# george-tyler-315-incline/ggml-neon-opt

Hardware: AMD Instinct MI355X
Metric: tg128 tok/s + Q4_K GEMV achieved-HBM-GB/s, TinyLlama-1.1B Q4_K_M @1 GPU (higher is better)
Workload: dtype q4_K/q6_K x q8_K (u4/u6*i8 dot4 -> i32, f32 combine); 1 GPU; tinyllama-1.1b Q4_K_M tg2221: full decode graph, token i at position i of a fresh f16 KV cache; parallelism=replicas x1, hipgraph=True

## Files before the change

ggml-neon-opt_amd/csrc/kq_backend.hip:

```cpp
#include <algorithm>
#include <dlfcn.h>
#include <stdio.h>
#include <stdlib.h>
#include <string.h>

#include <rccl/rccl.h>

#include <string>
#include <vector>

#include "kq_common.h"
#include "kq_internal.h"
#include "kq_plan.h"

using kq::attn_batch_desc_of;
using kq::attn_desc_of;
using kq::f_of;
using kq::Launch;
using kq::LaunchKind;
using kq::nelem;

struct mi355x_backend {
    int device = 0;
    hipStream_t stream = nullptr;
// ... 539 lines not shown
        }
        tb.stride = stride;
        tb.key.swap(key);
        b->ly_tabs.push_back(std::move(tb));
    }
    return MI355X_OK;
}

int reserve_attn_cells(mi355x_backend *b, mi355x_tensor *const *nodes, const std::vector<Launch> &launches) {
    for (const Launch &l : launches) {
        const mi355x_tensor *t = nodes[l.first];
        if (l.kind != LaunchKind::Node || t->op != MI355X_OP_ATTN_DECODE) continue;
        const int64_t T = t->src[0]->ne[1];
        mi355x_attn_desc d = {};
        attn_desc_of(t, d);
        if (T > 1) d.rope_row = 0;
        kq::AttnArgs a = {};
        if (kq::attn_args_from(&d, a) == MI355X_OK && kq::attn_cells_reserve(a, b->stream, (int)T) != MI355X_OK)
            return MI355X_E_WORKSPACE;
    }
    return MI355X_OK;
}

int capture_and_launch(mi355x_backend *b, mi355x_tensor *const *nodes, int n_nodes, const std::vector<Launch> &launches) {
    std::vector<uint64_t> key = kq::graph_key_of(nodes, n_nodes);
    mi355x_backend::Captured *c = find_graph(b, key);
    if (!c) {
        if (hipStreamBeginCapture(b->stream, hipStreamCaptureModeThreadLocal) != hipSuccess)
            return MI355X_E_UNSUPPORTED;
        const int rc = enqueue(b, nodes, launches);
        hipGraph_t g = nullptr;
        const hipError_t ec = hipStreamEndCapture(b->stream, &g);
        if (rc || ec != hipSuccess) {
            if (g) hipGraphDestroy(g);
            return rc ? rc : (int)ec;
        }
        hipGraphExec_t ge = nullptr;
        if (hipGraphInstantiate(&ge, g, nullptr, nullptr, 0) != hipSuccess) {
            hipGraphDestroy(g);
            return MI355X_E_UNSUPPORTED;
        }
        if (b->graphs.size() == kMaxGraphs) {
            hipStreamSynchronize(b->stream);
            destroy_captured(b->graphs.front());
            b->graphs.erase(b->graphs.begin());
        }
        mi355x_backend::Captured nc;
        nc.key.swap(key);
// ... 223 lines not shown
}

int mi355x_backend_set_fusion(mi355x_backend_t b, int enable) {
    return b ? toggle(b, b->fuse, enable) : MI355X_E_INVAL;
}

int mi355x_backend_graph_compute(mi355x_backend_t b, mi355x_tensor *const *nodes, int n_nodes, int use_graph) {
    if (!b || (n_nodes > 0 && !nodes) || n_nodes < 0) return MI355X_E_INVAL;
    DeviceGuard dg(b->device);
    if (use_graph && !b->graphs.empty()) {
        const std::vector<uint64_t> key = kq::graph_key_of(nodes, n_nodes);
        if (mi355x_backend::Captured *c = find_graph(b, key)) {
            const hipError_t e = hipGraphLaunch(c->exec, b->stream);
            return e == hipSuccess ? 0 : (int)e;
        }
    }
    int rc = ensure_workspace(b, nodes, n_nodes);
    if (rc) return rc;
    const std::vector<Launch> launches = kq::plan_launches(plan_opts(b), nodes, n_nodes);
    if ((rc = ensure_attn_oproj_buffer(b, nodes, launches))) return rc;
    if ((rc = ensure_layer_blocks(b, launches))) return rc;
    if ((rc = ensure_layer_tables(b, launches))) return rc;
    if ((rc = reserve_attn_cells(b, nodes, launches))) return rc;
    return use_graph ? capture_and_launch(b, nodes, n_nodes, launches) : enqueue(b, nodes, launches);
}

}
```

ggml-neon-opt_amd/csrc/kq_internal.h:

```cpp
#pragma once

#include <string>
#include <tuple>

#include <hip/hip_ext.h>

#include "kq_common.h"

namespace kq {

int device_ok();
int num_cus();
constexpr size_t kMaxLds = 160 * 1024;
constexpr size_t kTargetLds = 80 * 1024;
void allow_lds(const void *fn, size_t lds);
int resident_wgs(const void *fn, size_t lds);
uint64_t *diag_stamps(int64_t *cap);
enum Knob {
    KNOB_GEMV_DIAG,
    KNOB_GEMV_RING,
    KNOB_GEMV_PRE0,
    KNOB_GEMV_PF,
    KNOB_GEMV_XMODE,
    KNOB_GEMV_SMALL_MB,
// ... 125 lines not shown
int launch_mmf_multi(int type, int n_mat, const void *const *w, const int64_t *N, const size_t *row_stride,
                     float *const *y, const int64_t *y_col_stride, int64_t K, uint8_t *ws, size_t ws_size, int64_t M,
                     hipStream_t stream, const float *res = nullptr, int64_t res_col_stride = 0);
size_t mmf_workspace(int64_t N, int64_t M, int64_t nb);
struct MmqKv {
    int kind[4];
    const int32_t *pos;
    const float *rope;
    uint16_t *k_cache, *v_cache;
    int n_ctx, hd;
};
int launch_mmq_multi(const int *types, int n_mat, const void *const *w, const int64_t *N, const size_t *row_stride,
                     float *const *y, const int64_t *y_col_stride, int64_t K, const uint8_t *xq, int64_t M,
                     hipStream_t stream, const MmqKv *kv = nullptr);

int launch_rows_prologue_dbg(int pro, const float *x, const float *x2, float eps, int nb, int waves, uint8_t *out,
                             hipStream_t s);
int launch_rms_norm_q8L(const float *x, const float *w, void *yq, int64_t n, int64_t nrows, float eps, hipStream_t s);
int launch_swiglu_q8L(const float *g, const float *u, void *yq, int64_t n, int64_t nrows, hipStream_t s);

int launch_rms_norm(const float *x, const float *w, float *y, int64_t n, int64_t nrows, float eps, hipStream_t s);
int launch_binary(int op, const float *a, const float *b, float *y, int64_t n, hipStream_t s,
                  int64_t nb = 0);
int launch_attn_prompt(const AttnArgs &a, int n_tok, hipStream_t s);
int attn_cells_reserve(const AttnArgs &a, hipStream_t stream, int n_tok = 1);
bool attn_prompt_q8_ok(const AttnArgs &a);
int launch_swiglu(const float *g, const float *u, float *y, int64_t n, hipStream_t s);
int attn_args_from(const mi355x_attn_desc *d, AttnArgs &a);
int launch_attn(const AttnArgs &a, hipStream_t s);
bool attn_group_ok(const AttnArgs &a, int nwaves);
size_t attn_group_bytes(const AttnArgs &a, int nwaves);
int attn_impl();
size_t attn_lds(int hd, int n_ctx);
size_t attn_prompt_lds(int hd, int n_ctx);
void *attn_cells_buffer(size_t bytes, hipStream_t stream, bool may_alloc);
int launch_kv_store(const AttnArgs &a, int n_tok, hipStream_t s);

constexpr int kAttnStreamMaxCtx = 131072;
int attn_stream_mode();
bool attn_size_refused(const AttnArgs &a);
bool attn_stream_applies(const AttnArgs &a);
bool attn_stream_prompt_applies(const AttnArgs &a);
size_t attn_stream_workspace(const AttnArgs &a, int n_tok);
int launch_attn_stream(const AttnArgs &a, hipStream_t s);
int launch_attn_stream_prompt(const AttnArgs &a, int n_tok, hipStream_t s);

// ... 18 lines not shown
```

ggml-neon-opt_amd/csrc/kq_ops.hip:

```cpp
#include <math.h>
#include <stdlib.h>
#include <string.h>

#include <atomic>
#include <mutex>
#include <vector>

#include <hip/hip_ext.h>

#include "kq_common.h"
#include "kq_internal.h"
#include "kq_attn_device.h"
#include "kq_attn_head.h"
#include "kq_device.h"
#include "kq_ops_device.h"
#include "kq_rows_device.h"

#ifndef KQ_ATTN_BATCH_CTX
#define KQ_ATTN_BATCH_CTX 256
#endif
#ifndef KQ_ATTN_OSC1
#define KQ_ATTN_OSC1 0
#endif

namespace kq {

constexpr int GETROWS_STAGE = ((15 + 8 * 210 + 15) / 16) * 16;
__global__ void __launch_bounds__(256) kq_get_rows(int type, const uint8_t *__restrict__ table, int64_t k,
                                                   int64_t row_stride, int64_t n_rows,
                                                   const int32_t *__restrict__ ids, float *__restrict__ out) {
    __shared__ __attribute__((aligned(16))) uint8_t stage[GETROWS_STAGE];
    const int64_t r = blockIdx.y;
    const int64_t e0 = ((int64_t)blockIdx.x * 256 + threadIdx.x) * 8;
    const bool live = e0 < k;
    const int64_t id = ids[r];
    float *y = out + r * k + e0;
    if (id < 0 || id >= n_rows) {
        if (live) {
#pragma unroll
            for (int i = 0; i < 8; ++i) y[i] = __builtin_nanf("");
        }
        return;
    }
    const uint8_t *grow = table + id * row_stride;
    if (type == MI355X_TYPE_F32) {
        if (live) {
            const float *s = (const float *)grow + e0;
#pragma unroll
            for (int i = 0; i < 8; ++i) y[i] = s[i];
        }
        return;
    }
    const int bsz = block_bytes(type);
    const int64_t b0 = (int64_t)blockIdx.x * 8;
    const int64_t left = k / QK - b0;
    const int nblk = (int)(left < 8 ? left : 8);
    const uint8_t *src = grow + b0 * bsz;
    const uint32_t mis = (uint32_t)((uintptr_t)src & 15u);
    const int ng = (int)((mis + (uint32_t)(nblk * bsz) + 15u) / 16u);
// ... 24 lines not shown
        const uint8_t *qh = blk + 16 + l0;
#pragma unroll
        for (int i = 0; i < 8; ++i) {
            const int hb = q5 ? ((qh[i] >> (2 * j + h)) & 1) << 4 : 0;
            y[i] = __builtin_fmaf(d1, (float)(((q[i] >> (4 * h)) & 0xF) + hb), -m1);
        }
    } else {
        const uint8_t *blk = row + b * 210;
        const float d = h2f((uint16_t)(blk[208] | (blk[209] << 8)));
        const int half = e / 128, rr = e % 128, quarter = rr / 32, l0 = rr % 32;
        const uint8_t *ql = blk + 64 * half, *qh = blk + 128 + 32 * half;
        const int8_t *sc = (const int8_t *)(blk + 192) + 8 * half;
#pragma unroll
        for (int i = 0; i < 8; ++i) {
            const int l = l0 + i;
            int q;
            if (quarter == 0) q = (ql[l] & 0xF) | (((qh[l] >> 0) & 3) << 4);
            else if (quarter == 1) q = (ql[l + 32] & 0xF) | (((qh[l] >> 2) & 3) << 4);
            else if (quarter == 2) q = (ql[l] >> 4) | (((qh[l] >> 4) & 3) << 4);
            else q = (ql[l + 32] >> 4) | (((qh[l] >> 6) & 3) << 4);
            y[i] = d * (float)sc[l / 16 + 2 * quarter] * (float)(q - 32);
        }
    }
}

__global__ void __launch_bounds__(256) kq_rms_norm(const float *__restrict__ x, const float *__restrict__ w,
                                                   float *__restrict__ y, int64_t n, float eps) {
    extern __shared__ __attribute__((aligned(16))) double sb_sum[];
    const int64_t row = blockIdx.x;
    const float *xr = x + row * n;
    float *yr = y + row * n;
    const int nb = (int)(n / QK);
    const int rid = threadIdx.x >> 4, l = threadIdx.x & 15;
    for (int b0 = 0; b0 < nb; b0 += 16) {
        const int b = b0 + rid;
        double s = 0.0;
        if (b < nb) {
            float v[16];
            const float4 *p = (const float4 *)(xr + (int64_t)b * QK + 16 * l);
#pragma unroll
            for (int k = 0; k < 4; ++k) {
                const float4 t = p[k];
                v[4 * k] = t.x, v[4 * k + 1] = t.y, v[4 * k + 2] = t.z, v[4 * k + 3] = t.w;
            }
            s = sumsq16(v);
        }
// ... 1031 lines not shown
    if (rc) return rc;
    if (group) {
        if (gsz == 8 && tpw > 1) KQ_PROMPT_GROUP_LAUNCH(128, 8, KQ_PROMPT_TPW)
        if (gsz == 4 && tpw > 1) KQ_PROMPT_GROUP_LAUNCH(128, 4, KQ_PROMPT_TPW)
        if (gsz == 8) KQ_PROMPT_GROUP_LAUNCH(128, 8, 1)
        if (gsz == 4) KQ_PROMPT_GROUP_LAUNCH(128, 4, 1)
        KQ_PROMPT_GROUP_LAUNCH(128, 0, 1)
    }
#undef KQ_PROMPT_GROUP_LAUNCH
    allow_lds((const void *)kq_attn_prompt<128>, lds);
    return timed_launch("kq::kq_attn_prompt<128>", 0.0, kq_attn_prompt<128>, ga, dim3(256), lds, s, a);
}

int check_attn(const AttnArgs &a) {
    if (!a.q || !a.k || !a.v || !a.pos || !a.rope_table || !a.k_cache || !a.v_cache || !a.out) return MI355X_E_INVAL;
    if (a.head_dim != 64 && a.head_dim != 128) return MI355X_E_UNSUPPORTED;
    if (a.n_head <= 0 || a.n_head_kv <= 0 || a.n_head % a.n_head_kv) return MI355X_E_INVAL;
    if (a.n_ctx < 32 || a.n_ctx % 32) return MI355X_E_UNSUPPORTED;
    if (((uintptr_t)a.k_cache & 15u) || ((uintptr_t)a.v_cache & 15u)) return MI355X_E_INVAL;
    if (attn_size_refused(a) && !attn_stream_applies(a)) return MI355X_E_UNSUPPORTED;
    return MI355X_OK;
}

uint64_t ops_selector_key() {
    return (uint64_t)(uint32_t)attn_impl() | ((uint64_t)(uint32_t)g_prompt_impl.load() << 8) |
           ((uint64_t)(uint32_t)attn_stream_mode() << 16);
}

}

using namespace kq;

extern "C" {

int mi355x_get_rows(int type, const void *table, int64_t ne0, size_t row_stride, int64_t n_rows, const int32_t *ids,
                    int64_t n_ids, float *dst, void *stream) {
    if (!table || !ids || !dst || ne0 <= 0 || n_ids < 0 || n_rows < 0) return MI355X_E_INVAL;
    if (type != MI355X_TYPE_F32 && type != MI355X_TYPE_Q4_K && type != MI355X_TYPE_Q5_K && type != MI355X_TYPE_Q6_K)
        return MI355X_E_UNSUPPORTED;
    if (ne0 % (type == MI355X_TYPE_F32 ? 8 : QK)) return MI355X_E_INVAL;
    if (row_stride < mi355x_row_size(type, ne0) && type != MI355X_TYPE_F32) return MI355X_E_INVAL;
    if (n_ids == 0) return MI355X_OK;
    if (!device_ok()) return MI355X_E_NODEVICE;
    const dim3 grid((unsigned)((ne0 / 8 + 255) / 256), (unsigned)n_ids);
    return timed_launch("kq::kq_get_rows", (double)n_ids * (ne0 * 4.0 + (double)mi355x_row_size(type, ne0)),
                        kq_get_rows, grid, dim3(256), 0, (hipStream_t)stream, type, (const uint8_t *)table, ne0,
// ... 133 lines not shown
```

ggml-neon-opt_amd/csrc/kq_plan.h:

```cpp
#pragma once

#include <string.h>

#include <vector>

#include "kq_common.h"
#include "kq_internal.h"

namespace kq {

enum class LaunchKind {
    Node,
    GemvRun,
    PrefillPrologue,
    MmAdd,
    MmMulti,
    AttnOproj,
    Layer,
};

struct Launch {
    int first, count;
    LaunchKind kind = LaunchKind::Node;
    const mi355x_tensor *q8_of = nullptr;
// ... 13 lines not shown
    bool fuse, attn_oproj, layer_engine;
    const void *workspace;
    size_t workspace_size;
};

inline int64_t nelem(const mi355x_tensor *t) { return t->ne[0] * t->ne[1] * t->ne[2] * t->ne[3]; }
inline float f_of(int32_t bits) {
    float f;
    memcpy(&f, &bits, 4);
    return f;
}
inline const mi355x_tensor *other_operand(const mi355x_tensor *add, const mi355x_tensor *mm) {
    return add->src[0] == mm ? add->src[1] : add->src[1] == mm ? add->src[0] : nullptr;
}

std::vector<Launch> plan_launches(const PlanOpts &o, mi355x_tensor *const *nodes, int n);
bool batched_mm_shares(const PlanOpts &o, const mi355x_tensor *t);
bool attn_feeds_batched_mm(const PlanOpts &o, const mi355x_tensor *t, const Launch &next, mi355x_tensor *const *nodes);
bool kv_epilogue(mi355x_tensor *const *nodes, const Launch &l, const Launch &next, MmqKv &kv);
void attn_desc_of(const mi355x_tensor *t, mi355x_attn_desc &a);
void attn_batch_desc_of(const mi355x_tensor *t, mi355x_attn_batch_desc &d);
std::vector<uint64_t> graph_key_of(mi355x_tensor *const *nodes, int n_nodes);
bool supports_op(const mi355x_tensor *op);

}
```

ggml-neon-opt_amd/csrc/kq_plan.hip:

```cpp
#include "kq_plan.h"

namespace kq {
namespace {

bool is_kquant(int t) { return t == MI355X_TYPE_Q4_K || t == MI355X_TYPE_Q5_K || t == MI355X_TYPE_Q6_K; }

struct Span {
    uintptr_t lo = 0, hi = 0;
};
Span span_of(const mi355x_tensor *t) {
    Span s;
    if (!t || !t->data) return s;
    const int64_t blck = is_kquant(t->type) ? MI355X_QK_K : 1;
    uint64_t bytes = (uint64_t)(t->ne[0] / blck) * t->nb[0];
    for (int d = 1; d < 4; ++d)
        if (t->ne[d] > 1) bytes += (uint64_t)(t->ne[d] - 1) * t->nb[d];
    s.lo = (uintptr_t)t->data;
    s.hi = s.lo + (uintptr_t)bytes;
    return s;
}

std::vector<int> count_readers(mi355x_tensor *const *nodes, int n) {
    std::vector<int> r(n, 0);
    std::vector<Span> out(n);
// ... 450 lines not shown
    key.reserve((size_t)n_nodes * 16 + 2);
    key.push_back(api_selector_key());
    key.push_back(ops_selector_key());
    for (int i = 0; i < n_nodes; ++i) {
        const mi355x_tensor *t = nodes[i];
        key.push_back((uint64_t)(uintptr_t)t->data);
        key.push_back((uint64_t)t->op);
        key.push_back((uint64_t)t->flags);
        for (int d = 0; d < 4; ++d) key.push_back((uint64_t)t->ne[d]);
        for (int d = 0; d < 8; ++d) key.push_back((uint64_t)(uint32_t)t->op_params[d]);
        for (int s = 0; s < MI355X_MAX_SRC; ++s) {
            const mi355x_tensor *u = t->src[s];
            if (!u) { key.push_back(0); continue; }
            key.push_back((uint64_t)(uintptr_t)u->data);
            key.push_back((uint64_t)u->type);
            for (int d = 0; d < 4; ++d) key.push_back((uint64_t)u->ne[d]);
            for (int d = 0; d < 4; ++d) key.push_back((uint64_t)u->nb[d]);
        }
        for (int d = 0; d < 4; ++d) key.push_back((uint64_t)t->nb[d]);
    }
    return key;
}

bool supports_op(const mi355x_tensor *op) {
    if (!op) return false;
    switch (op->op) {
        case MI355X_OP_NONE:
            return true;
        case MI355X_OP_MUL_MAT: {
            const mi355x_tensor *w = op->src[0], *x = op->src[1];
            if (!w || !x) return false;
            if (!is_kquant(w->type) || x->type != MI355X_TYPE_F32 || op->type != MI355X_TYPE_F32) return false;
            if (w->ne[0] % MI355X_QK_K || w->ne[0] != x->ne[0]) return false;
            if (w->ne[2] != 1 || w->ne[3] != 1 || x->ne[2] != 1 || x->ne[3] != 1) return false;
            if (op->ne[0] != w->ne[1] || op->ne[1] != x->ne[1]) return false;
            if (x->nb[0] != 4 || op->nb[0] != 4) return false;
            return w->nb[0] == mi355x_row_size(w->type, MI355X_QK_K);
        }
        case MI355X_OP_GET_ROWS: {
            const mi355x_tensor *w = op->src[0], *ids = op->src[1];
            if (!w || !ids || ids->type != MI355X_TYPE_I32 || !ids->data || ids->nb[0] != 4 || !contig_f32(op))
                return false;
            if (w->type != MI355X_TYPE_F32 && !is_kquant(w->type)) return false;
            if (op->ne[1] > 1 && op->nb[1] != (size_t)op->ne[0] * 4) return false;
            return op->ne[0] == w->ne[0] && op->ne[1] == ids->ne[0] && w->ne[0] % MI355X_QK_K == 0;
        }
// ... 66 lines not shown
```

ggml-neon-opt_amd/ggml_mi355x/__init__.py:

```python
from __future__ import annotations

import ctypes
import os

HERE = os.path.dirname(os.path.abspath(__file__))
PKG_ROOT = os.path.dirname(HERE)
LIB_PATH = os.environ.get("MI355X_LIB") or os.path.join(PKG_ROOT, "lib", "libggml_mi355x.so")

TYPE_F32, TYPE_F16, TYPE_Q4_K, TYPE_Q5_K, TYPE_Q6_K, TYPE_Q8_K, TYPE_I32 = 0, 1, 12, 13, 14, 15, 26
TYPE_I64 = 27
QK_K = 256
BLOCK_BYTES = {TYPE_Q4_K: 144, TYPE_Q5_K: 176, TYPE_Q6_K: 210, TYPE_Q8_K: 292}
TYPE_NAMES = {TYPE_Q4_K: "q4_K", TYPE_Q5_K: "q5_K", TYPE_Q6_K: "q6_K", TYPE_Q8_K: "q8_K", TYPE_F32: "f32"}
MAX_FUSED = 4
OP_NONE, OP_MUL_MAT, OP_GET_ROWS, OP_RMS_NORM, OP_MUL, OP_ADD, OP_SWIGLU, OP_ROPE, OP_ATTN_DECODE, OP_ALL_GATHER, \
    OP_ALL_REDUCE = range(11)
OP_ATTN_BATCH = 11
MAX_SRC = 10
FLAG_OUTPUT = 1
E_OK, E_INVAL, E_UNSUPPORTED, E_WORKSPACE, E_NODEVICE, E_COMM, E_LAYER = 0, -1, -2, -3, -4, -6, -7
PRO_NONE, PRO_RMS_NORM, PRO_SWIGLU = 0, 1, 2
EPI_NONE, EPI_SWIGLU = 0, 1
ATTN_GROUP, ATTN_HEAD, ATTN_SPLIT = 0, 1, 2
ATTN_PATH_HEAD, ATTN_PATH_HEAD_BATCH, ATTN_PATH_SPLIT4, ATTN_PATH_SPLIT8, ATTN_PATH_CELLS, ATTN_PATH_GROUP, ATTN_PATH_KD1 = range(7)
ATTN_PATH_STREAM = 7
MMQ_AUTO, MMQ_TILE64, MMQ_TILE128, MMQ_TILE128W, MMQ_TILE64W, MMQ_TILE128X, MMQ_TILE192 = 0, 1, 2, 3, 4, 5, 6
PREFILL_EXACT, PREFILL_F16, PREFILL_F16_ALL = 0, 1, 2

EXPORTED_SYMBOLS = (
    "mi355x_row_size", "mi355x_version", "mi355x_device_available",
    "mi355x_quantize_row_q8_K", "mi355x_vec_dot_q4_K_q8_K", "mi355x_vec_dot_q5_K_q8_K",
    "mi355x_vec_dot_q6_K_q8_K", "mi355x_quantize_q8_K", "mi355x_mul_mat_workspace_size",
    "mi355x_mul_mat", "mi355x_mul_mat_q8", "mi355x_gemv_fused", "mi355x_debug_block_partials", "mi355x_debug_stream",
    "mi355x_backend_init", "mi355x_backend_free", "mi355x_backend_name", "mi355x_backend_stream",
    "mi355x_backend_alloc", "mi355x_backend_free_buffer", "mi355x_backend_set_tensor",
    "mi355x_backend_get_tensor", "mi355x_backend_synchronize", "mi355x_backend_supports_op",
    "mi355x_backend_graph_compute", "mi355x_timing_enable", "mi355x_timing_read", "mi355x_diag_stamps",
    "mi355x_gemv_fused_workspace_size", "mi355x_gemv_impl",
    "mi355x_gguf_open", "mi355x_gguf_close", "mi355x_gguf_version", "mi355x_gguf_alignment",
    "mi355x_gguf_data_offset", "mi355x_gguf_n_tensors", "mi355x_gguf_find_tensor", "mi355x_gguf_get_tensor",
    "mi355x_gguf_tensor_data", "mi355x_gguf_upload", "mi355x_gguf_n_kv", "mi355x_gguf_find_key",
    "mi355x_gguf_key", "mi355x_gguf_kv_type", "mi355x_gguf_get_int", "mi355x_gguf_get_float",
    "mi355x_gguf_get_str", "mi355x_gguf_arr_n",
    "mi355x_gemv_ext_workspace_size", "mi355x_gemv_fused_ext", "mi355x_backend_set_fusion",
    "mi355x_get_rows", "mi355x_rms_norm", "mi355x_add", "mi355x_mul", "mi355x_swiglu",
    "mi355x_rope_table_size", "mi355x_rope_table", "mi355x_rope", "mi355x_attn_decode", "mi355x_attn_path",
    "mi355x_comm_id_size", "mi355x_comm_get_unique_id", "mi355x_backend_set_comm", "mi355x_backend_comm_world",
    "mi355x_backend_set_comm_loopback", "mi355x_lower_ggml_graph", "mi355x_attn_impl",
    "mi355x_mmq_impl",
    "mi355x_prefill_precision",
    "mi355x_gemv_waves",
    "mi355x_debug_knob",
    "mi355x_device_count", "mi355x_device_ordinal", "mi355x_device_memory", "mi355x_backend_memset", "mi355x_backend_set_attn_oproj",
    "mi355x_backend_set_layer_engine", "mi355x_backend_layer_error",
    "mi355x_attn_prompt",
    "mi355x_attn_prompt_impl", "mi355x_attn_stream",
    "mi355x_attn_batch", "mi355x_attn_batch_path",
    "mi355x_rows_prologue_plan", "mi355x_rows_stream_plan", "mi355x_debug_rows_prologue",
    "mi355x_debug_rows_plan",
)


class Mi355xError(RuntimeError):
    pass


class GemvDesc(ctypes.Structure):
    _fields_ = [("type", ctypes.c_int), ("w", ctypes.c_void_p), ("n_rows", ctypes.c_int64),
                ("row_stride", ctypes.c_size_t), ("y", ctypes.c_void_p)]


class LaunchTiming(ctypes.Structure):
    _fields_ = [("kernel", ctypes.c_char * 96), ("bytes", ctypes.c_double), ("ms", ctypes.c_float)]


class Tensor(ctypes.Structure):
    pass


Tensor._fields_ = [("type", ctypes.c_int), ("op", ctypes.c_int), ("ne", ctypes.c_int64 * 4),
                   ("nb", ctypes.c_size_t * 4), ("src", ctypes.POINTER(Tensor) * MAX_SRC), ("data", ctypes.c_void_p),
                   ("op_params", ctypes.c_int32 * 8), ("flags", ctypes.c_int32)]
# ... 97 lines not shown
        L.mi355x_debug_rows_plan.restype = i32
    L.mi355x_debug_rows_prologue.argtypes = [i32, vp, vp, ctypes.c_float, i64, i32, vp, sz, vp]
    L.mi355x_debug_rows_prologue.restype = i32
    L.mi355x_backend_init.argtypes = [i32]
    L.mi355x_backend_init.restype = vp
    L.mi355x_backend_free.argtypes = [vp]
    L.mi355x_backend_name.argtypes = [vp]
    L.mi355x_backend_name.restype = ctypes.c_char_p
    L.mi355x_backend_stream.argtypes = [vp]
    L.mi355x_backend_stream.restype = vp
    L.mi355x_backend_alloc.argtypes = [vp, sz]
    L.mi355x_backend_alloc.restype = vp
    L.mi355x_backend_free_buffer.argtypes = [vp, vp]
    L.mi355x_backend_set_tensor.argtypes = [vp, vp, vp, sz]
    L.mi355x_backend_set_tensor.restype = i32
    L.mi355x_backend_get_tensor.argtypes = [vp, vp, vp, sz]
    L.mi355x_backend_get_tensor.restype = i32
    L.mi355x_backend_synchronize.argtypes = [vp]
    L.mi355x_backend_synchronize.restype = i32
    L.mi355x_backend_supports_op.argtypes = [ctypes.POINTER(Tensor)]
    L.mi355x_backend_supports_op.restype = i32
    L.mi355x_backend_graph_compute.argtypes = [vp, ctypes.POINTER(ctypes.POINTER(Tensor)), i32, i32]
    L.mi355x_backend_graph_compute.restype = i32
    L.mi355x_timing_enable.argtypes = [i32]
    L.mi355x_timing_enable.restype = i32
    L.mi355x_timing_read.argtypes = [ctypes.POINTER(LaunchTiming), i32]
    L.mi355x_timing_read.restype = i32
    L.mi355x_gemv_impl.argtypes = [i32]
    L.mi355x_gemv_impl.restype = i32
    L.mi355x_diag_stamps.argtypes = [vp, sz]
    L.mi355x_diag_stamps.restype = i32
    f32 = ctypes.c_float
    L.mi355x_gemv_ext_workspace_size.argtypes = [i64]
    L.mi355x_gemv_ext_workspace_size.restype = sz
    L.mi355x_gemv_fused_ext.argtypes = [ctypes.POINTER(GemvDesc), i32, vp, i64, ctypes.POINTER(GemvExt), vp, sz, vp]
    L.mi355x_gemv_fused_ext.restype = i32
    L.mi355x_backend_set_fusion.argtypes = [vp, i32]
    L.mi355x_backend_set_fusion.restype = i32
    L.mi355x_get_rows.argtypes = [i32, vp, i64, sz, i64, vp, i64, vp, vp]
    L.mi355x_rms_norm.argtypes = [vp, vp, vp, i64, i64, f32, vp]
    L.mi355x_add.argtypes = [vp, vp, vp, i64, vp]
    L.mi355x_mul.argtypes = [vp, vp, vp, i64, vp]
    L.mi355x_swiglu.argtypes = [vp, vp, vp, i64, vp]
    L.mi355x_rope_table_size.argtypes = [i32, i32]
    L.mi355x_rope_table_size.restype = sz
    L.mi355x_rope_table.argtypes = [vp, i32, i32, f32, f32, vp]
# ... 479 lines not shown
        return int(lib().mi355x_backend_set_attn_oproj(self.h, 1 if enable else 0))

    def set_layer_engine(self, enable):
        return int(lib().mi355x_backend_set_layer_engine(self.h, 1 if enable else 0))

    def layer_error(self):
        return int(lib().mi355x_backend_layer_error(self.h))

    def set_comm(self, rank, world, unique_id: bytes):
        buf = ctypes.create_string_buffer(bytes(unique_id), len(unique_id))
        _check(lib().mi355x_backend_set_comm(self.h, rank, world, buf), "set_comm")

    def set_comm_loopback(self, rank, world):
        _check(lib().mi355x_backend_set_comm_loopback(self.h, rank, world), "set_comm_loopback")

    @property
    def comm_world(self):
        return int(lib().mi355x_backend_comm_world(self.h))

    def graph_compute(self, nodes, use_graph=True):
        arr = (ctypes.POINTER(Tensor) * len(nodes))(*[ctypes.pointer(n) for n in nodes])
        return int(lib().mi355x_backend_graph_compute(self.h, arr, len(nodes), 1 if use_graph else 0))

    def close(self):
        if self.h:
            lib().mi355x_backend_free(self.h)
            self.h = None

    def __del__(self):
        try:
            self.close()
        except Exception:
            pass


def lower_ggml_graph(gnodes, rope_table_ptr, rope_n_pos, freq_base, freq_scale=1.0, arena_cap=None,
                     cells_eq_pos=True, cells_from_graph=False):
    n = len(gnodes)
    arr = (ctypes.POINTER(GTensor) * max(1, n))(*[ctypes.pointer(t) for t in gnodes])
    cap = arena_cap or (4 * n + 64)
    arena = (Tensor * cap)()
    out = (ctypes.POINTER(Tensor) * cap)()
    nn = ctypes.c_int(0)
    opts = LowerOpts(rope_table_ptr, rope_n_pos, freq_base, freq_scale, 1 if cells_eq_pos else 0,
                     1 if cells_from_graph else 0)
    rc = int(lib().mi355x_lower_ggml_graph(arr, n, ctypes.byref(opts), arena, cap, out, cap, ctypes.byref(nn)))
# ... 38 lines not shown
```

ggml-neon-opt_amd/ggml_mi355x/llama.py:

```python
from __future__ import annotations

import ctypes

from . import (FLAG_OUTPUT, OP_ADD, OP_ALL_GATHER, OP_ALL_REDUCE, OP_ATTN_BATCH, OP_ATTN_DECODE, OP_GET_ROWS, OP_MUL,
               OP_MUL_MAT,
               OP_RMS_NORM,
               OP_SWIGLU, TYPE_F16, TYPE_F32, TYPE_I32, Backend, Mi355xError, f32_bits, make_tensor, rope_table)

def torch_tensor(values):
    import torch
    return torch.tensor(list(values), dtype=torch.int32)


LAYER_MATS = ("attn_q", "attn_k", "attn_v", "attn_output", "ffn_gate", "ffn_up", "ffn_down")


def hparams(n_embd, n_layer, n_head, n_head_kv, n_ff, n_vocab, eps=1e-5, freq_base=10000.0):
    return dict(n_embd=n_embd, n_layer=n_layer, n_head=n_head, n_head_kv=n_head_kv, head_dim=n_embd // n_head,
                n_ff=n_ff, n_vocab=n_vocab, eps=eps, freq_base=freq_base)


TINYLLAMA = hparams(2048, 22, 32, 4, 5632, 32000)
LLAMA3_8B = hparams(4096, 32, 32, 8, 14336, 128256, eps=1e-5, freq_base=500000.0)


class LlamaDecoder:

    HOST_SLOTS = 1024
    BATCH_SLOTS = 64

    def __init__(self, backend: Backend, hp: dict, weights: dict, n_ctx: int, fuse: bool = True, split=None,
                 rope_src: str = "row"):
        import torch
        self.b, self.hp, self.w, self.n_ctx, self.split = backend, hp, weights, n_ctx, split
        dev = weights["output_norm"].device
        E, F, V = hp["n_embd"], hp["n_ff"], hp["n_vocab"]
        hd, nh, nkv = hp["head_dim"], hp["n_head"], hp["n_head_kv"]
        world = split.world if split is not None else 1
        if split is not None:
            nh, nkv = split.n_head, split.n_head_kv
        kvw = nkv * hd
        self.gathers = []
        self.reduces = []
        reduce_mode = split is not None and split.mode == "reduce"
        f32 = torch.float32

        def buf(n, dtype=f32):
            return torch.zeros(n, dtype=dtype, device=dev)

        self.inp = buf(2 + hd, torch.int32)
        self.token, self.pos = self.inp[0:1], self.inp[1:2]
# ... 94 lines not shown
                else:
                    db = self._bufs[-1]
                x, xb = allreduce(dn, db)
            else:
                glu, _ = gather(glu, F // world)
                dn = mm(p + "ffn_down", glu)
                res = ffn_inp if split is None else rows_view(fb, r_e0, El)
                x, xb = node(OP_ADD, El, [dn, res])
                x, xbg = gather(x, El)
                xb = xbg if xbg is not None else xb
            self.last_hidden = xb
        n3, _ = node(OP_RMS_NORM, E, [x], eps_bits)
        m3, _ = node(OP_MUL, E, [n3, leaf(weights["output_norm"], TYPE_F32, E)])
        wt = mat("output")
        if split is None:
            _, self.logits = node(OP_MUL_MAT, V, [wt, m3], flags=FLAG_OUTPUT)
        else:
            lg, _ = node(OP_MUL_MAT, wt.ne[1], [wt, m3])
            _, self.logits = gather(lg, V // world, flags=FLAG_OUTPUT)
        self._tensors = T
        self._arr = (ctypes.POINTER(type(T[0])) * len(self.nodes))(*[ctypes.pointer(n) for n in self.nodes])
        if backend is None:
            return
        self._host = torch.zeros((self.HOST_SLOTS, 2 + hd), dtype=torch.int32).pin_memory()
        self._slot = 0
        backend.set_fusion(fuse)
        torch.cuda.synchronize()

    def reset(self):
        for c in self.k_cache + self.v_cache:
            c.zero_()

    def _prompt_graph(self, n_tok: int):
        import torch
        cached = getattr(self, "_prompts", {}).get(n_tok)
        if cached is not None:
            return cached
        if self.split is not None:
            raise Mi355xError("prompt processing runs on one GPU (no row split)")
        hp, weights, n_ctx = self.hp, self.w, self.n_ctx
        dev = weights["output_norm"].device
        E, V = hp["n_embd"], hp["n_vocab"]
        hd, nh, nkv = hp["head_dim"], hp["n_head"], hp["n_head_kv"]
        kvw = nkv * hd
        T, bufs, nodes = [], [], []
        inp = torch.zeros(2 * n_tok + 1, dtype=torch.int32, device=dev)

        def leaf(t, type_, ne0, ne1=1, row_stride=None):
# ... 173 lines not shown
        m = torch.as_tensor(np.asarray(mask, dtype=np.float32) if not torch.is_tensor(mask) else mask).to(torch.float32)
        if m.dim() != 2 or m.shape[0] != n_tok or m.shape[1] < n_kv:
            raise Mi355xError(f"step_batch: mask must be [{n_tok}, >= {n_kv}]")
        from . import lib
        g = self._batch_graph(n_tok, n_kv)
        if g["slot"] == self.BATCH_SLOTS:
            self.b.synchronize()
            g["slot"] = 0
        host = g["host"][g["slot"]]
        g["slot"] += 1
        host[:n_tok] = torch_tensor(tokens)
        host[n_tok:2 * n_tok] = torch_tensor(pos)
        host[2 * n_tok:3 * n_tok] = torch_tensor(cells)
        host[3 * n_tok:].view(torch.float32).view(n_tok, n_kv).copy_(m[:, :n_kv])
        L = lib()
        rc = L.mi355x_backend_set_tensor(self.b.h, g["inp"].data_ptr(), host.data_ptr(), 4 * host.numel())
        if rc:
            raise Mi355xError(f"set_tensor failed ({rc})")
        rc = L.mi355x_backend_graph_compute(self.b.h, g["arr"], len(g["nodes"]), 1 if use_graph else 0)
        if rc:
            raise Mi355xError(f"graph_compute failed ({rc})")
        return g["logits"]

    def step(self, token: int, pos: int, use_graph: bool = True):
        if not 0 <= pos < self.n_ctx:
            raise Mi355xError(f"position {pos} outside the KV cache (n_ctx {self.n_ctx})")
        if not 0 <= token < self.hp["n_vocab"]:
            raise Mi355xError(f"token {token} outside the vocabulary (n_vocab {self.hp['n_vocab']})")
        from . import lib
        if self._slot == self.HOST_SLOTS:
            self.b.synchronize()
            self._slot = 0
        row = self._host[self._slot]
        row[0] = token
        row[1] = pos
        row[2:] = self._table_host[pos]
        L = lib()
        hp = row.data_ptr()
        self._slot += 1
        rc = L.mi355x_backend_set_tensor(self.b.h, self.inp.data_ptr(), hp, 4 * row.numel())
        if rc:
            raise Mi355xError(f"set_tensor failed ({rc})")
        rc = L.mi355x_backend_graph_compute(self.b.h, self._arr, len(self.nodes), 1 if use_graph else 0)
        if rc:
            raise Mi355xError(f"graph_compute failed ({rc})")
        return self.logits
```

include/ggml_mi355x.h:

```cpp
#ifndef GGML_MI355X_H
#define GGML_MI355X_H

#include <stddef.h>
#include <stdint.h>

#ifdef __cplusplus
extern "C" {
#endif

#define MI355X_QK_K 256
#define MI355X_K_SCALE_SIZE 12

typedef uint16_t mi355x_half;

typedef struct {
    mi355x_half d;
    mi355x_half dmin;
    uint8_t scales[MI355X_K_SCALE_SIZE];
    uint8_t qs[MI355X_QK_K / 2];
} mi355x_block_q4_K;

typedef struct {
    mi355x_half d;
    mi355x_half dmin;
// ... 205 lines not shown

int mi355x_device_count(void);
int mi355x_device_ordinal(int i);
int mi355x_device_memory(int device, size_t *free_bytes, size_t *total_bytes);
mi355x_backend_t mi355x_backend_init(int device);
void mi355x_backend_free(mi355x_backend_t backend);
const char *mi355x_backend_name(mi355x_backend_t backend);
void *mi355x_backend_stream(mi355x_backend_t backend);
void *mi355x_backend_alloc(mi355x_backend_t backend, size_t size);
void mi355x_backend_free_buffer(mi355x_backend_t backend, void *ptr);
int mi355x_backend_set_tensor(mi355x_backend_t backend, void *dst, const void *host_src,
                              size_t size);
int mi355x_backend_get_tensor(mi355x_backend_t backend, void *host_dst, const void *src,
                              size_t size);
int mi355x_backend_memset(mi355x_backend_t backend, void *dst, int value, size_t size);
int mi355x_backend_synchronize(mi355x_backend_t backend);
int mi355x_backend_supports_op(const mi355x_tensor *op);
int mi355x_backend_set_fusion(mi355x_backend_t backend, int enable);
int mi355x_backend_set_attn_oproj(mi355x_backend_t backend, int enable);
int mi355x_backend_set_layer_engine(mi355x_backend_t backend, int enable);
int mi355x_backend_layer_error(mi355x_backend_t backend);
int mi355x_backend_graph_compute(mi355x_backend_t backend, mi355x_tensor *const *nodes,
                                 int n_nodes, int use_graph);

enum mi355x_gop {
    MI355X_GOP_NONE = 0, MI355X_GOP_GET_ROWS, MI355X_GOP_RMS_NORM, MI355X_GOP_MUL, MI355X_GOP_ADD,
    MI355X_GOP_MUL_MAT, MI355X_GOP_ROPE, MI355X_GOP_SET_ROWS, MI355X_GOP_SOFT_MAX, MI355X_GOP_GLU,
    MI355X_GOP_RESHAPE, MI355X_GOP_VIEW, MI355X_GOP_PERMUTE, MI355X_GOP_TRANSPOSE, MI355X_GOP_CONT,
    MI355X_GOP_CPY,
};
#define MI355X_GLU_SWIGLU 2
typedef struct mi355x_gtensor {
    int type;
    int op;
    int64_t ne[4];
    size_t nb[4];
    int32_t op_params[16];
    int32_t flags;
    struct mi355x_gtensor *src[10];
    struct mi355x_gtensor *view_src;
    size_t view_offs;
    void *data;
    char name[64];
} mi355x_gtensor;
typedef struct {
    void *rope_table;
// ... 59 lines not shown
```

Before: 1559 tok/s.

## Fuse per-token input upload into the embedding get_rows kernel launch

Adds a graph_compute_inputs entry point. When the first node is a single-row get_rows, the per-token input words (token, pos, rope table) travel as kernel arguments to a new get_rows_in kernel. That kernel does the embedding lookup and writes the inputs buffer, then the captured graph of the remaining launches runs. This replaces the host-to-device memcpy of the pinned input row with one fused launch, cutting the copy and its per-step overhead. It adds a separately keyed graph and a 1 KB argument block per launch, and the step path stops using the pinned slot ring.

```diff
diff --git a/ggml-neon-opt_amd/csrc/kq_backend.hip b/ggml-neon-opt_amd/csrc/kq_backend.hip
--- a/ggml-neon-opt_amd/csrc/kq_backend.hip
+++ b/ggml-neon-opt_amd/csrc/kq_backend.hip
@@ -585,8 +585,8 @@
     return MI355X_OK;
 }
 
-int capture_and_launch(mi355x_backend *b, mi355x_tensor *const *nodes, int n_nodes, const std::vector<Launch> &launches) {
-    std::vector<uint64_t> key = kq::graph_key_of(nodes, n_nodes);
+int capture_and_launch(mi355x_backend *b, std::vector<uint64_t> key, mi355x_tensor *const *nodes,
+                       const std::vector<Launch> &launches) {
     mi355x_backend::Captured *c = find_graph(b, key);
     if (!c) {
         if (hipStreamBeginCapture(b->stream, hipStreamCaptureModeThreadLocal) != hipSuccess)
@@ -856,7 +856,62 @@
     if ((rc = ensure_layer_blocks(b, launches))) return rc;
     if ((rc = ensure_layer_tables(b, launches))) return rc;
     if ((rc = reserve_attn_cells(b, nodes, launches))) return rc;
-    return use_graph ? capture_and_launch(b, nodes, n_nodes, launches) : enqueue(b, nodes, launches);
-}
-
-}
+    return use_graph ? capture_and_launch(b, kq::graph_key_of(nodes, n_nodes), nodes, launches)
+                     : enqueue(b, nodes, launches);
+}
+
+int mi355x_inputs_path(mi355x_tensor *const *nodes, int n_nodes, const void *dst, size_t size) {
+    return kq::inputs_path(nodes, n_nodes, dst, size);
+}
+
+int mi355x_backend_graph_compute_inputs(mi355x_backend_t b, mi355x_tensor *const *nodes, int n_nodes, int use_graph,
+                                        void *dst, const void *host_src, size_t size) {
+    if (!b || (n_nodes > 0 && !nodes) || n_nodes < 0 || ((!dst || !host_src) && size)) return MI355X_E_INVAL;
+    std::vector<Launch> launches;
+    bool head = kq::inputs_path(nodes, n_nodes, dst, size) == MI355X_INPUTS_PATH_HEAD;
+    std::vector<uint64_t> key;
+    if (head) {
+        DeviceGuard dg(b->device);
+        const mi355x_tensor *t = nodes[0], *w = t->src[0];
+        const int32_t *words = (const int32_t *)host_src;
+        const int32_t id = words[((uintptr_t)t->src[1]->data - (uintptr_t)dst) / 4];
+        auto launch_head = [&] {
+            return kq::launch_get_rows_in(w->type, w->data, w->ne[0], w->nb[1], w->ne[1], id, (float *)t->data, dst,
+                                          host_src, size, b->stream);
+        };
+        if (use_graph) {
+            key = kq::graph_key_of(nodes, n_nodes);
+            key.push_back(kq::kInputsKeyMark);
+            if (mi355x_backend::Captured *c = b->graphs.empty() ? nullptr : find_graph(b, key)) {
+                const int rc = launch_head();
+                if (rc) return rc;
+                const hipError_t e = hipGraphLaunch(c->exec, b->stream);
+                return e == hipSuccess ? 0 : (int)e;
+            }
+        }
+        int rc = ensure_workspace(b, nodes, n_nodes);
+        if (rc) return rc;
+        launches = kq::plan_launches(plan_opts(b), nodes, n_nodes);
+        head = !launches.empty() && launches[0].kind == LaunchKind::Node && launches[0].first == 0 &&
+               launches[0].count == 1;
+        if (head) {
+            if ((rc = ensure_attn_oproj_buffer(b, nodes, launches))) return rc;
+            if ((rc = ensure_layer_blocks(b, launches))) return rc;
+            if ((rc = ensure_layer_tables(b, launches))) return rc;
+            if ((rc = reserve_attn_cells(b, nodes, launches))) return rc;
+            if ((rc = launch_head())) return rc;
+            launches.erase(launches.begin());
+            if (launches.empty()) return 0;
+            return use_graph ? capture_and_launch(b, std::move(key), nodes, launches) : enqueue(b, nodes, launches);
+        }
+    }
+    const int rc = mi355x_backend_set_tensor(b, dst, host_src, size);
+    if (rc) return rc;
+    if (size) {
+        DeviceGuard dg(b->device);
+        if (hipStreamSynchronize(b->stream) != hipSuccess) return MI355X_E_NODEVICE;
+    }
+    return mi355x_backend_graph_compute(b, nodes, n_nodes, use_graph);
+}
+
+}
diff --git a/ggml-neon-opt_amd/csrc/kq_internal.h b/ggml-neon-opt_amd/csrc/kq_internal.h
--- a/ggml-neon-opt_amd/csrc/kq_internal.h
+++ b/ggml-neon-opt_amd/csrc/kq_internal.h
@@ -171,6 +171,8 @@
 int launch_rms_norm(const float *x, const float *w, float *y, int64_t n, int64_t nrows, float eps, hipStream_t s);
 int launch_binary(int op, const float *a, const float *b, float *y, int64_t n, hipStream_t s,
                   int64_t nb = 0);
+int launch_get_rows_in(int type, const void *table, int64_t ne0, size_t row_stride, int64_t n_rows, int32_t id,
+                       float *dst_row, void *inputs, const void *host_src, size_t size, hipStream_t s);
 int launch_attn_prompt(const AttnArgs &a, int n_tok, hipStream_t s);
 int attn_cells_reserve(const AttnArgs &a, hipStream_t stream, int n_tok = 1);
 bool attn_prompt_q8_ok(const AttnArgs &a);
diff --git a/ggml-neon-opt_amd/csrc/kq_ops.hip b/ggml-neon-opt_amd/csrc/kq_ops.hip
--- a/ggml-neon-opt_amd/csrc/kq_ops.hip
+++ b/ggml-neon-opt_amd/csrc/kq_ops.hip
@@ -26,15 +26,12 @@
 namespace kq {
 
 constexpr int GETROWS_STAGE = ((15 + 8 * 210 + 15) / 16) * 16;
-__global__ void __launch_bounds__(256) kq_get_rows(int type, const uint8_t *__restrict__ table, int64_t k,
-                                                   int64_t row_stride, int64_t n_rows,
-                                                   const int32_t *__restrict__ ids, float *__restrict__ out) {
-    __shared__ __attribute__((aligned(16))) uint8_t stage[GETROWS_STAGE];
-    const int64_t r = blockIdx.y;
+__device__ __forceinline__ void get_rows_chunk(int type, const uint8_t *__restrict__ table, int64_t k,
+                                               int64_t row_stride, int64_t n_rows, int64_t id,
+                                               float *__restrict__ out_row, uint8_t *stage) {
     const int64_t e0 = ((int64_t)blockIdx.x * 256 + threadIdx.x) * 8;
     const bool live = e0 < k;
-    const int64_t id = ids[r];
-    float *y = out + r * k + e0;
+    float *y = out_row + e0;
     if (id < 0 || id >= n_rows) {
         if (live) {
 #pragma unroll
@@ -105,6 +102,30 @@
             y[i] = d * (float)sc[l / 16 + 2 * quarter] * (float)(q - 32);
         }
     }
+}
+
+__global__ void __launch_bounds__(256) kq_get_rows(int type, const uint8_t *__restrict__ table, int64_t k,
+                                                   int64_t row_stride, int64_t n_rows,
+                                                   const int32_t *__restrict__ ids, float *__restrict__ out) {
+    __shared__ __attribute__((aligned(16))) uint8_t stage[GETROWS_STAGE];
+    const int64_t r = blockIdx.y;
+    get_rows_chunk(type, table, k, row_stride, n_rows, ids[r], out + r * k, stage);
+}
+
+struct InputsBlock {
+    uint32_t w[MI355X_INPUTS_MAX / 4];
+};
+__global__ void __launch_bounds__(256) kq_get_rows_in(int type, const uint8_t *__restrict__ table, int64_t k,
+                                                      int64_t row_stride, int64_t n_rows, float *__restrict__ out,
+                                                      int id, int n_words, uint32_t *__restrict__ inputs,
+                                                      const InputsBlock blk) {
+    __shared__ __attribute__((aligned(16))) uint8_t stage[GETROWS_STAGE];
+    static_assert(MI355X_INPUTS_MAX / 4 <= 256, "one word per thread of the workgroup");
+    const bool carries = blockIdx.x == 0 && (int)threadIdx.x < n_words;
+    uint32_t word = 0;
+    if (carries) word = blk.w[threadIdx.x];
+    get_rows_chunk(type, table, k, row_stride, n_rows, id, out, stage);
+    if (carries) inputs[threadIdx.x] = word;
 }
 
 __global__ void __launch_bounds__(256) kq_rms_norm(const float *__restrict__ x, const float *__restrict__ w,
@@ -1182,6 +1203,24 @@
     return MI355X_OK;
 }
 
+int launch_get_rows_in(int type, const void *table, int64_t ne0, size_t row_stride, int64_t n_rows, int32_t id,
+                       float *dst_row, void *inputs, const void *host_src, size_t size, hipStream_t s) {
+    if (!table || !dst_row || !inputs || !host_src || ne0 <= 0 || n_rows < 0) return MI355X_E_INVAL;
+    if (!size || size % 4 || size > MI355X_INPUTS_MAX || ((uintptr_t)inputs & 3u)) return MI355X_E_INVAL;
+    if (type != MI355X_TYPE_F32 && type != MI355X_TYPE_Q4_K && type != MI355X_TYPE_Q5_K && type != MI355X_TYPE_Q6_K)
+        return MI355X_E_UNSUPPORTED;
+    if (ne0 % (type == MI355X_TYPE_F32 ? 8 : QK)) return MI355X_E_INVAL;
+    if (row_stride < mi355x_row_size(type, ne0) && type != MI355X_TYPE_F32) return MI355X_E_INVAL;
+    if (!device_ok()) return MI355X_E_NODEVICE;
+    InputsBlock blk;
+    memcpy(blk.w, host_src, size);
+    memset((uint8_t *)blk.w + size, 0, sizeof(blk.w) - size);
+    const dim3 grid((unsigned)((ne0 / 8 + 255) / 256));
+    return timed_launch("kq::kq_get_rows_in", ne0 * 4.0 + (double)mi355x_row_size(type, ne0) + (double)size,
+                        kq_get_rows_in, grid, dim3(256), 0, s, type, (const uint8_t *)table, ne0, (int64_t)row_stride,
+                        n_rows, dst_row, (int)id, (int)(size / 4), (uint32_t *)inputs, blk);
+}
+
 uint64_t ops_selector_key() {
     return (uint64_t)(uint32_t)attn_impl() | ((uint64_t)(uint32_t)g_prompt_impl.load() << 8) |
            ((uint64_t)(uint32_t)attn_stream_mode() << 16);
diff --git a/ggml-neon-opt_amd/csrc/kq_plan.h b/ggml-neon-opt_amd/csrc/kq_plan.h
--- a/ggml-neon-opt_amd/csrc/kq_plan.h
+++ b/ggml-neon-opt_amd/csrc/kq_plan.h
@@ -59,5 +59,7 @@
 void attn_batch_desc_of(const mi355x_tensor *t, mi355x_attn_batch_desc &d);
 std::vector<uint64_t> graph_key_of(mi355x_tensor *const *nodes, int n_nodes);
 bool supports_op(const mi355x_tensor *op);
+int inputs_path(mi355x_tensor *const *nodes, int n_nodes, const void *dst, size_t size);
+constexpr uint64_t kInputsKeyMark = 0x737475706e69ull;
 
 }
diff --git a/ggml-neon-opt_amd/csrc/kq_plan.hip b/ggml-neon-opt_amd/csrc/kq_plan.hip
--- a/ggml-neon-opt_amd/csrc/kq_plan.hip
+++ b/ggml-neon-opt_amd/csrc/kq_plan.hip
@@ -496,6 +496,22 @@
     return key;
 }
 
+int inputs_path(mi355x_tensor *const *nodes, int n_nodes, const void *dst, size_t size) {
+    if (!nodes || n_nodes < 1 || !dst || !size || size % 4 || size > MI355X_INPUTS_MAX) return MI355X_INPUTS_PATH_COPY;
+    if ((uintptr_t)dst & 3u) return MI355X_INPUTS_PATH_COPY;
+    const mi355x_tensor *t = nodes[0];
+    if (!t || t->op != MI355X_OP_GET_ROWS || !supports_op(t) || t->ne[1] != 1) return MI355X_INPUTS_PATH_COPY;
+    const mi355x_tensor *w = t->src[0], *ids = t->src[1];
+    if (w->type != MI355X_TYPE_F32 && w->type != MI355X_TYPE_Q4_K && w->type != MI355X_TYPE_Q5_K &&
+        w->type != MI355X_TYPE_Q6_K)
+        return MI355X_INPUTS_PATH_COPY;
+    if (!w->data || !t->data || (w->type != MI355X_TYPE_F32 && w->nb[1] < mi355x_row_size(w->type, w->ne[0])))
+        return MI355X_INPUTS_PATH_COPY;
+    const uintptr_t d0 = (uintptr_t)dst, id0 = (uintptr_t)ids->data;
+    if (id0 < d0 || id0 + 4 > d0 + size || (id0 - d0) % 4) return MI355X_INPUTS_PATH_COPY;
+    return MI355X_INPUTS_PATH_HEAD;
+}
+
 bool supports_op(const mi355x_tensor *op) {
     if (!op) return false;
     switch (op->op) {
diff --git a/ggml-neon-opt_amd/ggml_mi355x/__init__.py b/ggml-neon-opt_amd/ggml_mi355x/__init__.py
--- a/ggml-neon-opt_amd/ggml_mi355x/__init__.py
+++ b/ggml-neon-opt_amd/ggml_mi355x/__init__.py
@@ -24,6 +24,7 @@
 ATTN_GROUP, ATTN_HEAD, ATTN_SPLIT = 0, 1, 2
 ATTN_PATH_HEAD, ATTN_PATH_HEAD_BATCH, ATTN_PATH_SPLIT4, ATTN_PATH_SPLIT8, ATTN_PATH_CELLS, ATTN_PATH_GROUP, ATTN_PATH_KD1 = range(7)
 ATTN_PATH_STREAM = 7
+INPUTS_MAX, INPUTS_PATH_COPY, INPUTS_PATH_HEAD = 1024, 0, 1
 MMQ_AUTO, MMQ_TILE64, MMQ_TILE128, MMQ_TILE128W, MMQ_TILE64W, MMQ_TILE128X, MMQ_TILE192 = 0, 1, 2, 3, 4, 5, 6
 PREFILL_EXACT, PREFILL_F16, PREFILL_F16_ALL = 0, 1, 2
 
@@ -58,6 +59,7 @@
     "mi355x_attn_batch", "mi355x_attn_batch_path",
     "mi355x_rows_prologue_plan", "mi355x_rows_stream_plan", "mi355x_debug_rows_prologue",
     "mi355x_debug_rows_plan",
+    "mi355x_backend_graph_compute_inputs", "mi355x_inputs_path",
 )
 
 
@@ -201,6 +203,10 @@
     L.mi355x_backend_supports_op.restype = i32
     L.mi355x_backend_graph_compute.argtypes = [vp, ctypes.POINTER(ctypes.POINTER(Tensor)), i32, i32]
     L.mi355x_backend_graph_compute.restype = i32
+    L.mi355x_backend_graph_compute_inputs.argtypes = [vp, ctypes.POINTER(ctypes.POINTER(Tensor)), i32, i32, vp, vp, sz]
+    L.mi355x_backend_graph_compute_inputs.restype = i32
+    L.mi355x_inputs_path.argtypes = [ctypes.POINTER(ctypes.POINTER(Tensor)), i32, vp, sz]
+    L.mi355x_inputs_path.restype = i32
     L.mi355x_timing_enable.argtypes = [i32]
     L.mi355x_timing_enable.restype = i32
     L.mi355x_timing_read.argtypes = [ctypes.POINTER(LaunchTiming), i32]
@@ -726,6 +732,13 @@
         arr = (ctypes.POINTER(Tensor) * len(nodes))(*[ctypes.pointer(n) for n in nodes])
         return int(lib().mi355x_backend_graph_compute(self.h, arr, len(nodes), 1 if use_graph else 0))
 
+    def graph_compute_inputs(self, nodes, dst, host_array, use_graph=True):
+        import numpy as np
+        a = np.ascontiguousarray(host_array)
+        arr = (ctypes.POINTER(Tensor) * len(nodes))(*[ctypes.pointer(n) for n in nodes])
+        return int(lib().mi355x_backend_graph_compute_inputs(self.h, arr, len(nodes), 1 if use_graph else 0, dst,
+                                                             a.ctypes.data, a.nbytes))
+
     def close(self):
         if self.h:
             lib().mi355x_backend_free(self.h)
diff --git a/ggml-neon-opt_amd/ggml_mi355x/llama.py b/ggml-neon-opt_amd/ggml_mi355x/llama.py
--- a/ggml-neon-opt_amd/ggml_mi355x/llama.py
+++ b/ggml-neon-opt_amd/ggml_mi355x/llama.py
@@ -26,7 +26,6 @@
 
 class LlamaDecoder:
 
-    HOST_SLOTS = 1024
     BATCH_SLOTS = 64
 
     def __init__(self, backend: Backend, hp: dict, weights: dict, n_ctx: int, fuse: bool = True, split=None,
@@ -167,8 +166,7 @@
         self._arr = (ctypes.POINTER(type(T[0])) * len(self.nodes))(*[ctypes.pointer(n) for n in self.nodes])
         if backend is None:
             return
-        self._host = torch.zeros((self.HOST_SLOTS, 2 + hd), dtype=torch.int32).pin_memory()
-        self._slot = 0
+        self._row = torch.zeros(2 + hd, dtype=torch.int32)
         backend.set_fusion(fuse)
         torch.cuda.synchronize()
 
@@ -388,26 +386,45 @@
             raise Mi355xError(f"graph_compute failed ({rc})")
         return g["logits"]
 
+    EAGER_SLOTS = 1024
+
+    def _step_eager(self, token: int, pos: int):
+        import torch
+        from . import lib
+        if getattr(self, "_eager_host", None) is None:
+            self._eager_host = torch.zeros((self.EAGER_SLOTS, self.inp.numel()), dtype=torch.int32).pin_memory()
+            self._eager_slot = 0
+        if self._eager_slot == self.EAGER_SLOTS:
+            self.b.synchronize()
+            self._eager_slot = 0
+        row = self._eager_host[self._eager_slot]
+        self._eager_slot += 1
+        row[0] = token
+        row[1] = pos
+        row[2:] = self._table_host[pos]
+        L = lib()
+        rc = L.mi355x_backend_set_tensor(self.b.h, self.inp.data_ptr(), row.data_ptr(), 4 * row.numel())
+        if rc:
+            raise Mi355xError(f"set_tensor failed ({rc})")
+        rc = L.mi355x_backend_graph_compute(self.b.h, self._arr, len(self.nodes), 0)
+        if rc:
+            raise Mi355xError(f"graph_compute failed ({rc})")
+        return self.logits
+
     def step(self, token: int, pos: int, use_graph: bool = True):
         if not 0 <= pos < self.n_ctx:
             raise Mi355xError(f"position {pos} outside the KV cache (n_ctx {self.n_ctx})")
         if not 0 <= token < self.hp["n_vocab"]:
             raise Mi355xError(f"token {token} outside the vocabulary (n_vocab {self.hp['n_vocab']})")
         from . import lib
-        if self._slot == self.HOST_SLOTS:
-            self.b.synchronize()
-            self._slot = 0
-        row = self._host[self._slot]
+        if not use_graph:
+            return self._step_eager(token, pos)
+        row = self._row
         row[0] = token
         row[1] = pos
         row[2:] = self._table_host[pos]
-        L = lib()
-        hp = row.data_ptr()
-        self._slot += 1
-        rc = L.mi355x_backend_set_tensor(self.b.h, self.inp.data_ptr(), hp, 4 * row.numel())
-        if rc:
-            raise Mi355xError(f"set_tensor failed ({rc})")
-        rc = L.mi355x_backend_graph_compute(self.b.h, self._arr, len(self.nodes), 1 if use_graph else 0)
-        if rc:
-            raise Mi355xError(f"graph_compute failed ({rc})")
+        rc = lib().mi355x_backend_graph_compute_inputs(self.b.h, self._arr, len(self.nodes), 1 if use_graph else 0,
+                                                       self.inp.data_ptr(), row.data_ptr(), 4 * row.numel())
+        if rc:
+            raise Mi355xError(f"graph_compute_inputs failed ({rc})")
         return self.logits
diff --git a/include/ggml_mi355x.h b/include/ggml_mi355x.h
--- a/include/ggml_mi355x.h
+++ b/include/ggml_mi355x.h
@@ -251,6 +251,13 @@
 int mi355x_backend_layer_error(mi355x_backend_t backend);
 int mi355x_backend_graph_compute(mi355x_backend_t backend, mi355x_tensor *const *nodes,
                                  int n_nodes, int use_graph);
+#define MI355X_INPUTS_MAX 1024
+#define MI355X_INPUTS_PATH_COPY 0
+#define MI355X_INPUTS_PATH_HEAD 1
+int mi355x_backend_graph_compute_inputs(mi355x_backend_t backend, mi355x_tensor *const *nodes,
+                                        int n_nodes, int use_graph, void *dst,
+                                        const void *host_src, size_t size);
+int mi355x_inputs_path(mi355x_tensor *const *nodes, int n_nodes, const void *dst, size_t size);
 
 enum mi355x_gop {
     MI355X_GOP_NONE = 0, MI355X_GOP_GET_ROWS, MI355X_GOP_RMS_NORM, MI355X_GOP_MUL, MI355X_GOP_ADD,
```

Result: no change. 1568 tok/s (median of 6 runs) (+0.6%).
